# CPJKU/beat_this

Hardware: NVIDIA H100
Metric: clips/sec (30 s audio->beats, final0) (higher is better)
Workload: dtype f16

## Files before the change

beat_this_b200/csrc/kernels_attn.cu:

```cuda
#include <cstdio>
#include <type_traits>

#include "tc_common.cuh"

namespace bt {

constexpr int AT_BQ = 128;
constexpr int AT_BKV = 64;
constexpr int AT_NST = 4;
constexpr int AT_WARPS = 4;
constexpr int AT_RB = 2;
constexpr int AT_THREADS = 32 * AT_WARPS;
constexpr int AT_SQ = AT_BQ * 64;
constexpr int AT_SKV = AT_BKV * 64;
constexpr int AT_SMEM = 1024 + AT_SQ + AT_NST * 2 * AT_SKV + 128;
static_assert(AT_BQ == AT_WARPS * AT_RB * 16, "every query row of the tile belongs to one row block");

constexpr uint32_t AT_POLY_MASK = 0x52u;

__device__ __forceinline__ uint32_t sw64_off(int r, int c) {
  return static_cast<uint32_t>(r * 64 + ((c ^ ((r >> 1) & 3)) << 4));
}

__global__ void __launch_bounds__(AT_THREADS, 3)
attn_time_kernel(const __grid_constant__ CUtensorMap tmQ, const __grid_constant__ CUtensorMap tmKV,
                 const float* __restrict__ gates, h16* __restrict__ out, int L, int heads,
                 const ChunkSrc* __restrict__ chunks, int seqs_per_chunk) {
  extern __shared__ uint8_t smem_raw[];
  const uint32_t sbase = (smem_u32(smem_raw) + 1023u) & ~1023u;
  const uint32_t sQ = sbase;
  const uint32_t sK = sQ + AT_SQ;
  const uint32_t sV = sK + AT_NST * AT_SKV;
  const uint32_t bar_q = sV + AT_NST * AT_SKV;
  const uint32_t full = bar_q + 8;
  const uint32_t empty = full + 8 * AT_NST;

  const int warp = threadIdx.x >> 5, lane = threadIdx.x & 31;
  const int q0 = blockIdx.x * AT_BQ;
  const int h = blockIdx.y;
  const int seq = blockIdx.z;
  const int C = heads * 32;
  const int Lk = chunks ? chunks[seq / seqs_per_chunk].len : L;
  const int nkv = ceil_div(Lk, AT_BKV);

  if (threadIdx.x == 0) {
    mbar_init(bar_q, 1);
    for (int i = 0; i < AT_NST; ++i) {
      mbar_init(full + 8 * i, 1);
      mbar_init(empty + 8 * i, AT_WARPS);
    }
    fence_barrier_init();
  }
  __syncthreads();

  auto load_tile = [&](int t) {
    const int st = t % AT_NST;
    mbar_expect_tx(full + 8 * st, 2 * AT_SKV);
    tma_load_3d(sK + st * AT_SKV, &tmKV, full + 8 * st, C + h * 32, t * AT_BKV, seq);
    tma_load_3d(sV + st * AT_SKV, &tmKV, full + 8 * st, 2 * C + h * 32, t * AT_BKV, seq);
  };
  if (threadIdx.x == 0) {
    tma_prefetch_desc(&tmQ);
    tma_prefetch_desc(&tmKV);
    mbar_expect_tx(bar_q, AT_SQ);
    tma_load_3d(sQ, &tmQ, bar_q, h * 32, q0, seq);
    for (int t = 0; t < nkv && t < AT_NST; ++t) load_tile(t);
  }

  const int r0 = warp * (AT_RB * 16);
  mbar_wait(bar_q, 0);

  uint32_t qa[AT_RB][2][4];
#pragma unroll
  for (int b = 0; b < AT_RB; ++b)
#pragma unroll
    for (int ks = 0; ks < 2; ++ks)
      ldmatrix_x4(sQ + sw64_off(r0 + 16 * b + (lane & 15), 2 * ks + (lane >> 4)), qa[b][ks]);

  const uint32_t k_addr0 = sK + sw64_off(lane & 7, lane >> 3);
  const uint32_t v_addr0[2] = {sV + sw64_off(lane & 15, lane >> 4), sV + sw64_off(lane & 15, 2 + (lane >> 4))};
  const int key_lane = 2 * (lane & 3);

  float o[AT_RB][4][4];
#pragma unroll
  for (int b = 0; b < AT_RB; ++b)
#pragma unroll
    for (int d = 0; d < 4; ++d) o[b][d][0] = o[b][d][1] = o[b][d][2] = o[b][d][3] = 0.f;
  float m_run[AT_RB][2], l_run[AT_RB][2];
#pragma unroll
  for (int b = 0; b < AT_RB; ++b) m_run[b][0] = m_run[b][1] = -INFINITY, l_run[b][0] = l_run[b][1] = 0.f;
  auto kv_step = [&](uint32_t stage, uint32_t phase, auto last, int lim) {
    mbar_wait(full + stage / (AT_SKV / 8), phase);
    const uint32_t ka = k_addr0 + stage, va0 = v_addr0[0] + stage, va1 = v_addr0[1] + stage;
    float s[AT_RB][8][4];
#pragma unroll
    for (int nb = 0; nb < 8; ++nb) {
      uint32_t kf[4];
      ldmatrix_x4(ka + nb * 512, kf);
#pragma unroll
      for (int b = 0; b < AT_RB; ++b) {
        s[b][nb][0] = s[b][nb][1] = s[b][nb][2] = s[b][nb][3] = 0.f;
        mma_16816(s[b][nb], qa[b][0], kf[0], kf[1]);
        mma_16816(s[b][nb], qa[b][1], kf[2], kf[3]);
      }
    }
    if constexpr (decltype(last)::value) {
#pragma unroll
      for (int nb = 0; nb < 8; ++nb) {
        const int key = nb * 8 + key_lane;
#pragma unroll
        for (int b = 0; b < AT_RB; ++b) {
          if (key >= lim) s[b][nb][0] = s[b][nb][2] = -INFINITY;
          if (key + 1 >= lim) s[b][nb][1] = s[b][nb][3] = -INFINITY;
        }
      }
    }
    float mref[AT_RB][2];
#pragma unroll
    for (int b = 0; b < AT_RB; ++b) {
      float mx[2];
#pragma unroll
      for (int r = 0; r < 2; ++r) {
        float t[8];
#pragma unroll
        for (int nb = 0; nb < 8; ++nb) t[nb] = fmaxf(s[b][nb][2 * r], s[b][nb][2 * r + 1]);
#pragma unroll
        for (int w = 4; w > 0; w >>= 1)
#pragma unroll
          for (int i = 0; i < w; ++i) t[i] = fmaxf(t[i], t[i + w]);
        mx[r] = t[0];
      }
      float alpha[2];
#pragma unroll
      for (int r = 0; r < 2; ++r) {
        mx[r] = fmaxf(mx[r], __shfl_xor_sync(0xffffffffu, mx[r], 1));
        mx[r] = fmaxf(mx[r], __shfl_xor_sync(0xffffffffu, mx[r], 2));
        mref[b][r] = fmaxf(m_run[b][r], mx[r]);
        alpha[r] = ex2_approx(m_run[b][r] - mref[b][r]);
        m_run[b][r] = mref[b][r];
        l_run[b][r] *= alpha[r];
      }
#pragma unroll
      for (int d = 0; d < 4; ++d) {
        o[b][d][0] *= alpha[0]; o[b][d][1] *= alpha[0];
        o[b][d][2] *= alpha[1]; o[b][d][3] *= alpha[1];
      }
    }
    uint32_t pa[AT_RB][4][4];
#pragma unroll
    for (int b = 0; b < AT_RB; ++b)
#pragma unroll
      for (int nb = 0; nb < 8; ++nb) {
        float p[4];
#pragma unroll
        for (int i = 0; i < 4; ++i) {
          const float x = s[b][nb][i] - mref[b][i >> 1];
          p[i] = ((AT_POLY_MASK >> nb) & 1u) ? ex2_poly(x) : ex2_approx(x);
        }
        l_run[b][0] += p[0] + p[1];
        l_run[b][1] += p[2] + p[3];
        pa[b][nb >> 1][(nb & 1) * 2] = pack_h16x2(p[0], p[1]);
        pa[b][nb >> 1][(nb & 1) * 2 + 1] = pack_h16x2(p[2], p[3]);
      }
#pragma unroll
    for (int kk = 0; kk < 4; ++kk) {
#pragma unroll
      for (int dp = 0; dp < 2; ++dp) {
        uint32_t vf[4];
        ldmatrix_x4_trans((dp ? va1 : va0) + kk * 1024, vf);
#pragma unroll
        for (int b = 0; b < AT_RB; ++b) {
          mma_16816(o[b][2 * dp], pa[b][kk], vf[0], vf[1]);
          mma_16816(o[b][2 * dp + 1], pa[b][kk], vf[2], vf[3]);
        }
      }
    }
    __syncwarp();
    if (lane == 0) mbar_arrive(empty + stage / (AT_SKV / 8));
  };
  uint32_t stage = 0, phase = 0;
  for (int j = 0; j < nkv - 1; ++j) {
    if (threadIdx.x == 0 && j > 0 && j + AT_NST - 1 < nkv) {
      mbar_wait(empty + 8 * ((j - 1) % AT_NST), ((j - 1) / AT_NST) & 1);
      load_tile(j + AT_NST - 1);
    }
    kv_step(stage, phase, std::false_type{}, 0);
    stage += AT_SKV;
    if (stage == AT_NST * AT_SKV) stage = 0, phase ^= 1;
  }
  if (nkv > 0) kv_step(stage, phase, std::true_type{}, Lk - (nkv - 1) * AT_BKV);
#pragma unroll
  for (int b = 0; b < AT_RB; ++b)
#pragma unroll
    for (int r = 0; r < 2; ++r) {
      l_run[b][r] += __shfl_xor_sync(0xffffffffu, l_run[b][r], 1);
      l_run[b][r] += __shfl_xor_sync(0xffffffffu, l_run[b][r], 2);
    }
#pragma unroll
  for (int b = 0; b < AT_RB; ++b)
#pragma unroll
    for (int r = 0; r < 2; ++r) {
      const int q = q0 + r0 + 16 * b + (lane >> 2) + 8 * r;
      if (q < L) {
        const int64_t m = static_cast<int64_t>(seq) * L + q;
        const float gsc = gates[m * heads + h] / l_run[b][r];
        h16* dst = out + m * C + h * 32 + 2 * (lane & 3);
#pragma unroll
        for (int d = 0; d < 4; ++d)
          *reinterpret_cast<uint32_t*>(dst + 8 * d) = pack_h16x2(o[b][d][2 * r] * gsc, o[b][d][2 * r + 1] * gsc);
      }
    }
}

struct TcAttnPlan {
  CUtensorMap tmQ;
  CUtensorMap tmKV;
  int seqs, L, heads;
};

TcAttnPlan* tc_attn_plan_create(const void* qkv, int seqs, int L, int heads, char* err, int errlen) {
  TcAttnPlan* p = new TcAttnPlan();
  p->seqs = seqs; p->L = L; p->heads = heads;
  const int C = heads * 32;
  const uint64_t dims[3] = {static_cast<uint64_t>(3 * C), static_cast<uint64_t>(L), static_cast<uint64_t>(seqs)};
  const uint64_t strides[2] = {static_cast<uint64_t>(3 * C) * 2, static_cast<uint64_t>(L) * 3 * C * 2};
  const uint32_t box_q[3] = {32, AT_BQ, 1};
  const uint32_t box_kv[3] = {32, AT_BKV, 1};
  if (!make_tmap(&p->tmQ, qkv, 3, dims, strides, box_q, 64, err, errlen) ||
      !make_tmap(&p->tmKV, qkv, 3, dims, strides, box_kv, 64, err, errlen)) {
    delete p;
    return nullptr;
  }
  return p;
}
void tc_attn_plan_destroy(TcAttnPlan* p) { delete p; }

void launch_attn_time_tc(const TcAttnPlan* p, const float* gates, void* out, cudaStream_t st, const ChunkSrc* chunks,
                         int seqs_per_chunk) {
  dim3 grid(ceil_div(p->L, AT_BQ), p->heads, p->seqs);
  attn_time_kernel<<<grid, AT_THREADS, AT_SMEM, st>>>(p->tmQ, p->tmKV, gates, reinterpret_cast<h16*>(out), p->L, p->heads,
                                                      chunks, seqs_per_chunk);
}

int tc_init_attn(char* err, int errlen) {
  const cudaError_t r = cudaFuncSetAttribute(attn_time_kernel, cudaFuncAttributeMaxDynamicSharedMemorySize, AT_SMEM);
  if (r != cudaSuccess) {
    snprintf(err, errlen, "cudaFuncSetAttribute(attn_time_kernel) failed: %s", cudaGetErrorString(r));
    return -1;
  }
  return 0;
}

}
```

beat_this_b200/csrc/tc_common.cuh:

```cuda
#pragma once
#include <cuda.h>

#include "epilogue.cuh"

namespace bt {

__device__ __forceinline__ void tma_store_3d(const void* tmap, uint32_t smem_src, int32_t c0, int32_t c1, int32_t c2) {
  asm volatile("cp.async.bulk.tensor.3d.global.shared::cta.bulk_group [%0, {%2, %3, %4}], [%1];" ::"l"(
                   reinterpret_cast<uint64_t>(tmap)),
               "r"(smem_src), "r"(c0), "r"(c1), "r"(c2)
               : "memory");
}
__device__ __forceinline__ void bulk_commit() { asm volatile("cp.async.bulk.commit_group;" ::: "memory"); }
template <int N>
__device__ __forceinline__ void bulk_wait_read() {
  asm volatile("cp.async.bulk.wait_group.read %0;" ::"n"(N) : "memory");
}
__device__ __forceinline__ void named_bar_sync(int id, int count) {
  asm volatile("bar.sync %0, %1;" ::"r"(id), "r"(count) : "memory");
}
__device__ __forceinline__ void stmatrix_x4(uint32_t addr, uint32_t r0, uint32_t r1, uint32_t r2, uint32_t r3) {
  asm volatile("stmatrix.sync.aligned.m8n8.x4.shared.b16 [%0], {%1, %2, %3, %4};" ::"r"(addr), "r"(r0), "r"(r1), "r"(r2),
               "r"(r3)
               : "memory");
}
__device__ __forceinline__ float2 ld_shared_v2_f32(uint32_t addr) {
  float2 q;
  asm volatile("ld.shared.v2.f32 {%0, %1}, [%2];" : "=f"(q.x), "=f"(q.y) : "r"(addr) : "memory");
  return q;
}
__device__ __forceinline__ void st_shared_v2_f32(uint32_t addr, float x, float y) {
  asm volatile("st.shared.v2.f32 [%0], {%1, %2};" ::"r"(addr), "f"(x), "f"(y) : "memory");
}

__device__ __forceinline__ float ex2_approx(float x) {
  float y;
  asm("ex2.approx.ftz.f32 %0, %1;" : "=f"(y) : "f"(x));
  return y;
}
__device__ __forceinline__ float ex2_poly(float x) {
  x = fmaxf(x, -120.0f);
  const float magic = 12582912.0f;
  const float t = x + magic;
  const float r = x - (t - magic);
  float p = fmaf(0.05508868f, r, 0.24260405f);
  p = fmaf(p, r, 0.69327623f);
  p = fmaf(p, r, 0.99992895f);
  int y;
  asm("mad.lo.s32 %0, %1, 8388608, %2;" : "=r"(y) : "r"(__float_as_int(t)), "r"(__float_as_int(p)));
  return __int_as_float(y);
}

template <int SW>
__device__ __forceinline__ uint64_t make_wgmma_desc(uint32_t smem_addr) {
  static_assert(SW == 128 || SW == 64, "swizzle");
  constexpr uint64_t layout = SW == 128 ? 1 : 2;
  constexpr uint64_t sbo = (8 * SW) >> 4;
  return static_cast<uint64_t>((smem_addr & 0x3FFFF) >> 4) | (1ull << 16) | (sbo << 32) | (layout << 62);
}
__device__ __forceinline__ void wgmma_fence() { asm volatile("wgmma.fence.sync.aligned;" ::: "memory"); }
__device__ __forceinline__ void wgmma_commit() { asm volatile("wgmma.commit_group.sync.aligned;" ::: "memory"); }
template <int N>
__device__ __forceinline__ void wgmma_wait() {
  asm volatile("wgmma.wait_group.sync.aligned %0;" ::"n"(N) : "memory");
}
template <int R>
__device__ __forceinline__ void setmaxnreg_dec() {
  asm volatile("setmaxnreg.dec.sync.aligned.u32 %0;" ::"n"(R));
}
template <int R>
__device__ __forceinline__ void setmaxnreg_inc() {
  asm volatile("setmaxnreg.inc.sync.aligned.u32 %0;" ::"n"(R));
}
template <int N>
__device__ __forceinline__ void wgmma_m64k16(float (&d)[N / 2], uint64_t a_desc, uint64_t b_desc, uint32_t accumulate) {
  static_assert(N == 32 || N == 64 || N == 128 || N == 192 || N == 256, "wgmma width");
  if constexpr (N == 32) {
    asm volatile(
        "{\n\t.reg .pred p;\n\tsetp.ne.b32 p, %18, 0;\n\t"
        "wgmma.mma_async.sync.aligned.m64n32k16.f32." BT_H16_MMA_SYNC " "
        "{%0, %1, %2, %3, %4, %5, %6, %7, %8, %9, %10, %11, %12, %13, %14, %15}, "
        "%16, %17, p, 1, 1, 0, 0;\n\t}"
        : "+f"(d[0]), "+f"(d[1]), "+f"(d[2]), "+f"(d[3]), "+f"(d[4]), "+f"(d[5]), "+f"(d[6]), "+f"(d[7]),
          "+f"(d[8]), "+f"(d[9]), "+f"(d[10]), "+f"(d[11]), "+f"(d[12]), "+f"(d[13]), "+f"(d[14]), "+f"(d[15])
        : "l"(a_desc), "l"(b_desc), "r"(accumulate)
        : "memory");
  } else if constexpr (N == 64) {
    asm volatile(
        "{\n\t.reg .pred p;\n\tsetp.ne.b32 p, %34, 0;\n\t"
        "wgmma.mma_async.sync.aligned.m64n64k16.f32." BT_H16_MMA_SYNC " "
        "{%0, %1, %2, %3, %4, %5, %6, %7, %8, %9, %10, %11, %12, %13, %14, %15, %16, %17, %18, %19, %20, %21, %22, %23, %24, %25, %26, %27, %28, %29, %30, %31}, "
        "%32, %33, p, 1, 1, 0, 0;\n\t}"
        : "+f"(d[0]), "+f"(d[1]), "+f"(d[2]), "+f"(d[3]), "+f"(d[4]), "+f"(d[5]), "+f"(d[6]), "+f"(d[7]),
          "+f"(d[8]), "+f"(d[9]), "+f"(d[10]), "+f"(d[11]), "+f"(d[12]), "+f"(d[13]), "+f"(d[14]), "+f"(d[15]),
          "+f"(d[16]), "+f"(d[17]), "+f"(d[18]), "+f"(d[19]), "+f"(d[20]), "+f"(d[21]), "+f"(d[22]), "+f"(d[23]),
          "+f"(d[24]), "+f"(d[25]), "+f"(d[26]), "+f"(d[27]), "+f"(d[28]), "+f"(d[29]), "+f"(d[30]), "+f"(d[31])
        : "l"(a_desc), "l"(b_desc), "r"(accumulate)
        : "memory");
  } else if constexpr (N == 128) {
    asm volatile(
        "{\n\t.reg .pred p;\n\tsetp.ne.b32 p, %66, 0;\n\t"
        "wgmma.mma_async.sync.aligned.m64n128k16.f32." BT_H16_MMA_SYNC " "
        "{%0, %1, %2, %3, %4, %5, %6, %7, %8, %9, %10, %11, %12, %13, %14, %15, %16, %17, %18, %19, %20, %21, %22, %23, %24, %25, %26, %27, %28, %29, %30, %31, %32, %33, %34, %35, %36, %37, %38, %39, %40, %41, %42, %43, %44, %45, %46, %47, %48, %49, %50, %51, %52, %53, %54, %55, %56, %57, %58, %59, %60, %61, %62, %63}, "
        "%64, %65, p, 1, 1, 0, 0;\n\t}"
        : "+f"(d[0]), "+f"(d[1]), "+f"(d[2]), "+f"(d[3]), "+f"(d[4]), "+f"(d[5]), "+f"(d[6]), "+f"(d[7]),
          "+f"(d[8]), "+f"(d[9]), "+f"(d[10]), "+f"(d[11]), "+f"(d[12]), "+f"(d[13]), "+f"(d[14]), "+f"(d[15]),
          "+f"(d[16]), "+f"(d[17]), "+f"(d[18]), "+f"(d[19]), "+f"(d[20]), "+f"(d[21]), "+f"(d[22]), "+f"(d[23]),
          "+f"(d[24]), "+f"(d[25]), "+f"(d[26]), "+f"(d[27]), "+f"(d[28]), "+f"(d[29]), "+f"(d[30]), "+f"(d[31]),
          "+f"(d[32]), "+f"(d[33]), "+f"(d[34]), "+f"(d[35]), "+f"(d[36]), "+f"(d[37]), "+f"(d[38]), "+f"(d[39]),
          "+f"(d[40]), "+f"(d[41]), "+f"(d[42]), "+f"(d[43]), "+f"(d[44]), "+f"(d[45]), "+f"(d[46]), "+f"(d[47]),
          "+f"(d[48]), "+f"(d[49]), "+f"(d[50]), "+f"(d[51]), "+f"(d[52]), "+f"(d[53]), "+f"(d[54]), "+f"(d[55]),
          "+f"(d[56]), "+f"(d[57]), "+f"(d[58]), "+f"(d[59]), "+f"(d[60]), "+f"(d[61]), "+f"(d[62]), "+f"(d[63])
        : "l"(a_desc), "l"(b_desc), "r"(accumulate)
        : "memory");
  } else if constexpr (N == 192) {
    asm volatile(
        "{\n\t.reg .pred p;\n\tsetp.ne.b32 p, %98, 0;\n\t"
        "wgmma.mma_async.sync.aligned.m64n192k16.f32." BT_H16_MMA_SYNC " "
        "{%0, %1, %2, %3, %4, %5, %6, %7, %8, %9, %10, %11, %12, %13, %14, %15, %16, %17, %18, %19, %20, %21, %22, %23, %24, %25, %26, %27, %28, %29, %30, %31, %32, %33, %34, %35, %36, %37, %38, %39, %40, %41, %42, %43, %44, %45, %46, %47, %48, %49, %50, %51, %52, %53, %54, %55, %56, %57, %58, %59, %60, %61, %62, %63, %64, %65, %66, %67, %68, %69, %70, %71, %72, %73, %74, %75, %76, %77, %78, %79, %80, %81, %82, %83, %84, %85, %86, %87, %88, %89, %90, %91, %92, %93, %94, %95}, "
        "%96, %97, p, 1, 1, 0, 0;\n\t}"
        : "+f"(d[0]), "+f"(d[1]), "+f"(d[2]), "+f"(d[3]), "+f"(d[4]), "+f"(d[5]), "+f"(d[6]), "+f"(d[7]),
          "+f"(d[8]), "+f"(d[9]), "+f"(d[10]), "+f"(d[11]), "+f"(d[12]), "+f"(d[13]), "+f"(d[14]), "+f"(d[15]),
          "+f"(d[16]), "+f"(d[17]), "+f"(d[18]), "+f"(d[19]), "+f"(d[20]), "+f"(d[21]), "+f"(d[22]), "+f"(d[23]),
          "+f"(d[24]), "+f"(d[25]), "+f"(d[26]), "+f"(d[27]), "+f"(d[28]), "+f"(d[29]), "+f"(d[30]), "+f"(d[31]),
          "+f"(d[32]), "+f"(d[33]), "+f"(d[34]), "+f"(d[35]), "+f"(d[36]), "+f"(d[37]), "+f"(d[38]), "+f"(d[39]),
          "+f"(d[40]), "+f"(d[41]), "+f"(d[42]), "+f"(d[43]), "+f"(d[44]), "+f"(d[45]), "+f"(d[46]), "+f"(d[47]),
          "+f"(d[48]), "+f"(d[49]), "+f"(d[50]), "+f"(d[51]), "+f"(d[52]), "+f"(d[53]), "+f"(d[54]), "+f"(d[55]),
          "+f"(d[56]), "+f"(d[57]), "+f"(d[58]), "+f"(d[59]), "+f"(d[60]), "+f"(d[61]), "+f"(d[62]), "+f"(d[63]),
          "+f"(d[64]), "+f"(d[65]), "+f"(d[66]), "+f"(d[67]), "+f"(d[68]), "+f"(d[69]), "+f"(d[70]), "+f"(d[71]),
          "+f"(d[72]), "+f"(d[73]), "+f"(d[74]), "+f"(d[75]), "+f"(d[76]), "+f"(d[77]), "+f"(d[78]), "+f"(d[79]),
          "+f"(d[80]), "+f"(d[81]), "+f"(d[82]), "+f"(d[83]), "+f"(d[84]), "+f"(d[85]), "+f"(d[86]), "+f"(d[87]),
          "+f"(d[88]), "+f"(d[89]), "+f"(d[90]), "+f"(d[91]), "+f"(d[92]), "+f"(d[93]), "+f"(d[94]), "+f"(d[95])
        : "l"(a_desc), "l"(b_desc), "r"(accumulate)
        : "memory");
  } else if constexpr (N == 256) {
    asm volatile(
        "{\n\t.reg .pred p;\n\tsetp.ne.b32 p, %130, 0;\n\t"
        "wgmma.mma_async.sync.aligned.m64n256k16.f32." BT_H16_MMA_SYNC " "
        "{%0, %1, %2, %3, %4, %5, %6, %7, %8, %9, %10, %11, %12, %13, %14, %15, %16, %17, %18, %19, %20, %21, %22, %23, %24, %25, %26, %27, %28, %29, %30, %31, %32, %33, %34, %35, %36, %37, %38, %39, %40, %41, %42, %43, %44, %45, %46, %47, %48, %49, %50, %51, %52, %53, %54, %55, %56, %57, %58, %59, %60, %61, %62, %63, %64, %65, %66, %67, %68, %69, %70, %71, %72, %73, %74, %75, %76, %77, %78, %79, %80, %81, %82, %83, %84, %85, %86, %87, %88, %89, %90, %91, %92, %93, %94, %95, %96, %97, %98, %99, %100, %101, %102, %103, %104, %105, %106, %107, %108, %109, %110, %111, %112, %113, %114, %115, %116, %117, %118, %119, %120, %121, %122, %123, %124, %125, %126, %127}, "
        "%128, %129, p, 1, 1, 0, 0;\n\t}"
        : "+f"(d[0]), "+f"(d[1]), "+f"(d[2]), "+f"(d[3]), "+f"(d[4]), "+f"(d[5]), "+f"(d[6]), "+f"(d[7]),
          "+f"(d[8]), "+f"(d[9]), "+f"(d[10]), "+f"(d[11]), "+f"(d[12]), "+f"(d[13]), "+f"(d[14]), "+f"(d[15]),
          "+f"(d[16]), "+f"(d[17]), "+f"(d[18]), "+f"(d[19]), "+f"(d[20]), "+f"(d[21]), "+f"(d[22]), "+f"(d[23]),
          "+f"(d[24]), "+f"(d[25]), "+f"(d[26]), "+f"(d[27]), "+f"(d[28]), "+f"(d[29]), "+f"(d[30]), "+f"(d[31]),
          "+f"(d[32]), "+f"(d[33]), "+f"(d[34]), "+f"(d[35]), "+f"(d[36]), "+f"(d[37]), "+f"(d[38]), "+f"(d[39]),
          "+f"(d[40]), "+f"(d[41]), "+f"(d[42]), "+f"(d[43]), "+f"(d[44]), "+f"(d[45]), "+f"(d[46]), "+f"(d[47]),
          "+f"(d[48]), "+f"(d[49]), "+f"(d[50]), "+f"(d[51]), "+f"(d[52]), "+f"(d[53]), "+f"(d[54]), "+f"(d[55]),
          "+f"(d[56]), "+f"(d[57]), "+f"(d[58]), "+f"(d[59]), "+f"(d[60]), "+f"(d[61]), "+f"(d[62]), "+f"(d[63]),
          "+f"(d[64]), "+f"(d[65]), "+f"(d[66]), "+f"(d[67]), "+f"(d[68]), "+f"(d[69]), "+f"(d[70]), "+f"(d[71]),
          "+f"(d[72]), "+f"(d[73]), "+f"(d[74]), "+f"(d[75]), "+f"(d[76]), "+f"(d[77]), "+f"(d[78]), "+f"(d[79]),
          "+f"(d[80]), "+f"(d[81]), "+f"(d[82]), "+f"(d[83]), "+f"(d[84]), "+f"(d[85]), "+f"(d[86]), "+f"(d[87]),
          "+f"(d[88]), "+f"(d[89]), "+f"(d[90]), "+f"(d[91]), "+f"(d[92]), "+f"(d[93]), "+f"(d[94]), "+f"(d[95]),
          "+f"(d[96]), "+f"(d[97]), "+f"(d[98]), "+f"(d[99]), "+f"(d[100]), "+f"(d[101]), "+f"(d[102]), "+f"(d[103]),
          "+f"(d[104]), "+f"(d[105]), "+f"(d[106]), "+f"(d[107]), "+f"(d[108]), "+f"(d[109]), "+f"(d[110]), "+f"(d[111]),
          "+f"(d[112]), "+f"(d[113]), "+f"(d[114]), "+f"(d[115]), "+f"(d[116]), "+f"(d[117]), "+f"(d[118]), "+f"(d[119]),
          "+f"(d[120]), "+f"(d[121]), "+f"(d[122]), "+f"(d[123]), "+f"(d[124]), "+f"(d[125]), "+f"(d[126]), "+f"(d[127])
        : "l"(a_desc), "l"(b_desc), "r"(accumulate)
        : "memory");
  }
}

__device__ __forceinline__ void mma_16816(float (&d)[4], const uint32_t (&a)[4], uint32_t b0, uint32_t b1) {
  asm volatile("mma.sync.aligned.m16n8k16.row.col.f32." BT_H16_MMA_SYNC ".f32 {%0, %1, %2, %3}, {%4, %5, %6, %7}, {%8, %9}, "
               "{%0, %1, %2, %3};"
               : "+f"(d[0]), "+f"(d[1]), "+f"(d[2]), "+f"(d[3])
               : "r"(a[0]), "r"(a[1]), "r"(a[2]), "r"(a[3]), "r"(b0), "r"(b1));
}
__device__ __forceinline__ void ldmatrix_x4(uint32_t addr, uint32_t (&r)[4]) {
  asm volatile("ldmatrix.sync.aligned.m8n8.x4.shared.b16 {%0, %1, %2, %3}, [%4];"
               : "=r"(r[0]), "=r"(r[1]), "=r"(r[2]), "=r"(r[3])
               : "r"(addr)
               : "memory");
}
__device__ __forceinline__ void ldmatrix_x4_trans(uint32_t addr, uint32_t (&r)[4]) {
  asm volatile("ldmatrix.sync.aligned.m8n8.x4.trans.shared.b16 {%0, %1, %2, %3}, [%4];"
               : "=r"(r[0]), "=r"(r[1]), "=r"(r[2]), "=r"(r[3])
               : "r"(addr)
               : "memory");
}

extern int g_num_sms;
bool make_tmap(CUtensorMap* tm, const void* base, int rank, const uint64_t* dims, const uint64_t* strides_bytes,
               const uint32_t* box, int swizzle_bytes, char* err, int errlen);
int tc_init_attn(char* err, int errlen);
int tc_init_attn_freq(char* err, int errlen);
int tc_init_fused(char* err, int errlen);

}
```

Baseline: 815.7.

## Port time-attention kernel from mma.sync to pipelined wgmma warpgroups

Rewrites the flash-attention time kernel to use two warpgroups issuing asynchronous wgmma, computing QK^T from shared-memory descriptors and PV with register-sourced P. Score MMAs for the next KV tile are issued before the softmax of the current one, so tensor-core work overlaps the exponentials. The empty-barrier release moves to one arrival per warpgroup, and the final division uses a custom f64-refined reciprocal. This adds register pressure from double-buffered scores and depends on the wgmma descriptor and swizzle layout matching the TMA layout.

```diff
diff --git a/beat_this_b200/csrc/kernels_attn.cu b/beat_this_b200/csrc/kernels_attn.cu
--- a/beat_this_b200/csrc/kernels_attn.cu
+++ b/beat_this_b200/csrc/kernels_attn.cu
@@ -8,21 +8,35 @@
 constexpr int AT_BQ = 128;
 constexpr int AT_BKV = 64;
 constexpr int AT_NST = 4;
-constexpr int AT_WARPS = 4;
-constexpr int AT_RB = 2;
-constexpr int AT_THREADS = 32 * AT_WARPS;
+constexpr int AT_WG = 2;
+constexpr int AT_THREADS = 128 * AT_WG;
 constexpr int AT_SQ = AT_BQ * 64;
 constexpr int AT_SKV = AT_BKV * 64;
 constexpr int AT_SMEM = 1024 + AT_SQ + AT_NST * 2 * AT_SKV + 128;
-static_assert(AT_BQ == AT_WARPS * AT_RB * 16, "every query row of the tile belongs to one row block");
+static_assert(AT_BQ == AT_WG * 64, "every query row of the tile belongs to one warpgroup");
 
 constexpr uint32_t AT_POLY_MASK = 0x52u;
 
-__device__ __forceinline__ uint32_t sw64_off(int r, int c) {
-  return static_cast<uint32_t>(r * 64 + ((c ^ ((r >> 1) & 3)) << 4));
-}
-
-__global__ void __launch_bounds__(AT_THREADS, 3)
+__device__ __forceinline__ float div_rn_nocall(float a, float b) {
+  const double ad = a, bd = b;
+  double y;
+  asm("rcp.approx.ftz.f64 %0, %1;" : "=d"(y) : "d"(bd));
+  y = fma(y, fma(-bd, y, 1.0), y);
+  y = fma(y, fma(-bd, y, 1.0), y);
+  const double q = ad * y;
+  return static_cast<float>(fma(fma(-bd, q, ad), y, q));
+}
+
+__device__ __forceinline__ void mbar_wait_asm(uint32_t bar, uint32_t parity) {
+  asm volatile(
+      "{\n\t.reg .pred p;\n\tWAIT_%=:\n\t"
+      "mbarrier.try_wait.parity.shared::cta.b64 p, [%0], %1;\n\t"
+      "@!p bra WAIT_%=;\n\t}" ::"r"(bar),
+      "r"(parity)
+      : "memory");
+}
+
+__global__ void __launch_bounds__(AT_THREADS, 2)
 attn_time_kernel(const __grid_constant__ CUtensorMap tmQ, const __grid_constant__ CUtensorMap tmKV,
                  const float* __restrict__ gates, h16* __restrict__ out, int L, int heads,
                  const ChunkSrc* __restrict__ chunks, int seqs_per_chunk) {
@@ -35,7 +49,8 @@
   const uint32_t full = bar_q + 8;
   const uint32_t empty = full + 8 * AT_NST;
 
-  const int warp = threadIdx.x >> 5, lane = threadIdx.x & 31;
+  const int wg = threadIdx.x >> 7, warp = (threadIdx.x >> 5) & 3, lane = threadIdx.x & 31;
+  const bool leader = (threadIdx.x & 127) == 0;
   const int q0 = blockIdx.x * AT_BQ;
   const int h = blockIdx.y;
   const int seq = blockIdx.z;
@@ -47,7 +62,7 @@
     mbar_init(bar_q, 1);
     for (int i = 0; i < AT_NST; ++i) {
       mbar_init(full + 8 * i, 1);
-      mbar_init(empty + 8 * i, AT_WARPS);
+      mbar_init(empty + 8 * i, AT_WG);
     }
     fence_barrier_init();
   }
@@ -67,149 +82,141 @@
     for (int t = 0; t < nkv && t < AT_NST; ++t) load_tile(t);
   }
 
-  const int r0 = warp * (AT_RB * 16);
+  const uint32_t sQw = sQ + wg * 64 * 64;
+  const int key_lane = 2 * (lane & 3);
   mbar_wait(bar_q, 0);
 
-  uint32_t qa[AT_RB][2][4];
-#pragma unroll
-  for (int b = 0; b < AT_RB; ++b)
-#pragma unroll
-    for (int ks = 0; ks < 2; ++ks)
-      ldmatrix_x4(sQ + sw64_off(r0 + 16 * b + (lane & 15), 2 * ks + (lane >> 4)), qa[b][ks]);
-
-  const uint32_t k_addr0 = sK + sw64_off(lane & 7, lane >> 3);
-  const uint32_t v_addr0[2] = {sV + sw64_off(lane & 15, lane >> 4), sV + sw64_off(lane & 15, 2 + (lane >> 4))};
-  const int key_lane = 2 * (lane & 3);
-
-  float o[AT_RB][4][4];
-#pragma unroll
-  for (int b = 0; b < AT_RB; ++b)
-#pragma unroll
-    for (int d = 0; d < 4; ++d) o[b][d][0] = o[b][d][1] = o[b][d][2] = o[b][d][3] = 0.f;
-  float m_run[AT_RB][2], l_run[AT_RB][2];
-#pragma unroll
-  for (int b = 0; b < AT_RB; ++b) m_run[b][0] = m_run[b][1] = -INFINITY, l_run[b][0] = l_run[b][1] = 0.f;
-  auto kv_step = [&](uint32_t stage, uint32_t phase, auto last, int lim) {
-    mbar_wait(full + stage / (AT_SKV / 8), phase);
-    const uint32_t ka = k_addr0 + stage, va0 = v_addr0[0] + stage, va1 = v_addr0[1] + stage;
-    float s[AT_RB][8][4];
-#pragma unroll
-    for (int nb = 0; nb < 8; ++nb) {
-      uint32_t kf[4];
-      ldmatrix_x4(ka + nb * 512, kf);
-#pragma unroll
-      for (int b = 0; b < AT_RB; ++b) {
-        s[b][nb][0] = s[b][nb][1] = s[b][nb][2] = s[b][nb][3] = 0.f;
-        mma_16816(s[b][nb], qa[b][0], kf[0], kf[1]);
-        mma_16816(s[b][nb], qa[b][1], kf[2], kf[3]);
-      }
-    }
-    if constexpr (decltype(last)::value) {
+  float s[2][32], o[16];
+#pragma unroll
+  for (int i = 0; i < 16; ++i) asm volatile("mov.b32 %0, 0;" : "=f"(o[i]));
+  uint32_t pa[2][4][4];
+  float m_run[2] = {-INFINITY, -INFINITY}, l_run[2] = {0.f, 0.f};
+
+  const uint64_t qdesc = make_wgmma_desc<64>(sQw), kdesc = make_wgmma_desc<64>(sK);
+  auto issue_scores = [&](float (&acc)[32], uint32_t stage) {
+    wgmma_fence();
+    wgmma_m64n64k16_zero(acc, qdesc, kdesc + (stage >> 4));
+    wgmma_m64k16<64>(acc, qdesc + 2, kdesc + (stage >> 4) + 2, 1u);
+  };
+  auto kv_step = [&](int j, uint32_t stage, uint32_t phase, auto B, auto last, int lim) {
+    constexpr int b = decltype(B)::value;
+    constexpr bool is_last = decltype(last)::value;
+    if constexpr (!is_last) {
+      const uint32_t next = stage + AT_SKV == AT_NST * AT_SKV ? 0u : stage + AT_SKV;
+      mbar_wait(full + next / (AT_SKV / 8), next == 0 ? phase ^ 1u : phase);
+      issue_scores(s[b ^ 1], next);
+      wgmma_commit();
+    }
+    wgmma_wait<is_last ? 1 : 2>();
+    wgmma_fence_operands(s[b]);
+    if constexpr (is_last) {
 #pragma unroll
       for (int nb = 0; nb < 8; ++nb) {
         const int key = nb * 8 + key_lane;
-#pragma unroll
-        for (int b = 0; b < AT_RB; ++b) {
-          if (key >= lim) s[b][nb][0] = s[b][nb][2] = -INFINITY;
-          if (key + 1 >= lim) s[b][nb][1] = s[b][nb][3] = -INFINITY;
-        }
-      }
-    }
-    float mref[AT_RB][2];
-#pragma unroll
-    for (int b = 0; b < AT_RB; ++b) {
-      float mx[2];
-#pragma unroll
-      for (int r = 0; r < 2; ++r) {
-        float t[8];
-#pragma unroll
-        for (int nb = 0; nb < 8; ++nb) t[nb] = fmaxf(s[b][nb][2 * r], s[b][nb][2 * r + 1]);
-#pragma unroll
-        for (int w = 4; w > 0; w >>= 1)
-#pragma unroll
-          for (int i = 0; i < w; ++i) t[i] = fmaxf(t[i], t[i + w]);
-        mx[r] = t[0];
-      }
-      float alpha[2];
-#pragma unroll
-      for (int r = 0; r < 2; ++r) {
-        mx[r] = fmaxf(mx[r], __shfl_xor_sync(0xffffffffu, mx[r], 1));
-        mx[r] = fmaxf(mx[r], __shfl_xor_sync(0xffffffffu, mx[r], 2));
-        mref[b][r] = fmaxf(m_run[b][r], mx[r]);
-        alpha[r] = ex2_approx(m_run[b][r] - mref[b][r]);
-        m_run[b][r] = mref[b][r];
-        l_run[b][r] *= alpha[r];
-      }
-#pragma unroll
-      for (int d = 0; d < 4; ++d) {
-        o[b][d][0] *= alpha[0]; o[b][d][1] *= alpha[0];
-        o[b][d][2] *= alpha[1]; o[b][d][3] *= alpha[1];
-      }
-    }
-    uint32_t pa[AT_RB][4][4];
-#pragma unroll
-    for (int b = 0; b < AT_RB; ++b)
-#pragma unroll
-      for (int nb = 0; nb < 8; ++nb) {
-        float p[4];
-#pragma unroll
-        for (int i = 0; i < 4; ++i) {
-          const float x = s[b][nb][i] - mref[b][i >> 1];
-          p[i] = ((AT_POLY_MASK >> nb) & 1u) ? ex2_poly(x) : ex2_approx(x);
-        }
-        l_run[b][0] += p[0] + p[1];
-        l_run[b][1] += p[2] + p[3];
-        pa[b][nb >> 1][(nb & 1) * 2] = pack_h16x2(p[0], p[1]);
-        pa[b][nb >> 1][(nb & 1) * 2 + 1] = pack_h16x2(p[2], p[3]);
-      }
-#pragma unroll
-    for (int kk = 0; kk < 4; ++kk) {
-#pragma unroll
-      for (int dp = 0; dp < 2; ++dp) {
-        uint32_t vf[4];
-        ldmatrix_x4_trans((dp ? va1 : va0) + kk * 1024, vf);
-#pragma unroll
-        for (int b = 0; b < AT_RB; ++b) {
-          mma_16816(o[b][2 * dp], pa[b][kk], vf[0], vf[1]);
-          mma_16816(o[b][2 * dp + 1], pa[b][kk], vf[2], vf[3]);
-        }
-      }
+        if (key >= lim) s[b][4 * nb] = s[b][4 * nb + 2] = -INFINITY;
+        if (key + 1 >= lim) s[b][4 * nb + 1] = s[b][4 * nb + 3] = -INFINITY;
+      }
+    }
+    float mref[2], alpha[2];
+#pragma unroll
+    for (int r = 0; r < 2; ++r) {
+      float t[8];
+#pragma unroll
+      for (int nb = 0; nb < 8; ++nb) t[nb] = fmaxf(s[b][4 * nb + 2 * r], s[b][4 * nb + 2 * r + 1]);
+#pragma unroll
+      for (int w = 4; w > 0; w >>= 1)
+#pragma unroll
+        for (int i = 0; i < w; ++i) t[i] = fmaxf(t[i], t[i + w]);
+      float mx = t[0];
+      mx = fmaxf(mx, __shfl_xor_sync(0xffffffffu, mx, 1));
+      mx = fmaxf(mx, __shfl_xor_sync(0xffffffffu, mx, 2));
+      mref[r] = fmaxf(m_run[r], mx);
+      alpha[r] = ex2_approx(m_run[r] - mref[r]);
+      m_run[r] = mref[r];
+      l_run[r] *= alpha[r];
+    }
+    wgmma_wait<is_last ? 0 : 1>();
+    wgmma_fence_operands(o);
+    if (leader && j > 0) mbar_arrive(empty + 8 * ((j - 1) % AT_NST));
+#pragma unroll
+    for (int d = 0; d < 4; ++d) {
+      o[4 * d] *= alpha[0]; o[4 * d + 1] *= alpha[0];
+      o[4 * d + 2] *= alpha[1]; o[4 * d + 3] *= alpha[1];
+    }
+#pragma unroll
+    for (int nb = 0; nb < 8; ++nb) {
+      float p[4];
+#pragma unroll
+      for (int i = 0; i < 4; ++i) {
+        const float x = s[b][4 * nb + i] - mref[i >> 1];
+        p[i] = ((AT_POLY_MASK >> nb) & 1u) ? ex2_poly(x) : ex2_approx(x);
+      }
+      l_run[0] += p[0] + p[1];
+      l_run[1] += p[2] + p[3];
+      pa[b][nb >> 1][(nb & 1) * 2] = pack_h16x2(p[0], p[1]);
+      pa[b][nb >> 1][(nb & 1) * 2 + 1] = pack_h16x2(p[2], p[3]);
+    }
+    wgmma_fence_operands(o);
+#pragma unroll
+    for (int kk = 0; kk < 4; ++kk) wgmma_fence_operands(pa[b][kk]);
+    wgmma_fence();
+#pragma unroll
+    for (int kk = 0; kk < 4; ++kk)
+      wgmma_m64n32k16_rs_tb(o, pa[b][kk], kdesc + ((AT_NST * AT_SKV + stage + kk * 1024) >> 4));
+    wgmma_commit();
+    if constexpr (is_last) {
+      wgmma_wait<0>();
+      wgmma_fence_operands(o);
+    }
+    if (threadIdx.x == 0 && j > 0 && j + AT_NST - 1 < nkv) {
+      mbar_wait_asm(empty + 8 * ((j - 1) % AT_NST), ((j - 1) / AT_NST) & 1);
+      load_tile(j + AT_NST - 1);
     }
     __syncwarp();
-    if (lane == 0) mbar_arrive(empty + stage / (AT_SKV / 8));
   };
-  uint32_t stage = 0, phase = 0;
-  for (int j = 0; j < nkv - 1; ++j) {
-    if (threadIdx.x == 0 && j > 0 && j + AT_NST - 1 < nkv) {
-      mbar_wait(empty + 8 * ((j - 1) % AT_NST), ((j - 1) / AT_NST) & 1);
-      load_tile(j + AT_NST - 1);
-    }
-    kv_step(stage, phase, std::false_type{}, 0);
-    stage += AT_SKV;
-    if (stage == AT_NST * AT_SKV) stage = 0, phase ^= 1;
-  }
-  if (nkv > 0) kv_step(stage, phase, std::true_type{}, Lk - (nkv - 1) * AT_BKV);
-#pragma unroll
-  for (int b = 0; b < AT_RB; ++b)
-#pragma unroll
-    for (int r = 0; r < 2; ++r) {
-      l_run[b][r] += __shfl_xor_sync(0xffffffffu, l_run[b][r], 1);
-      l_run[b][r] += __shfl_xor_sync(0xffffffffu, l_run[b][r], 2);
-    }
-#pragma unroll
-  for (int b = 0; b < AT_RB; ++b)
-#pragma unroll
-    for (int r = 0; r < 2; ++r) {
-      const int q = q0 + r0 + 16 * b + (lane >> 2) + 8 * r;
-      if (q < L) {
-        const int64_t m = static_cast<int64_t>(seq) * L + q;
-        const float gsc = gates[m * heads + h] / l_run[b][r];
-        h16* dst = out + m * C + h * 32 + 2 * (lane & 3);
-#pragma unroll
-        for (int d = 0; d < 4; ++d)
-          *reinterpret_cast<uint32_t*>(dst + 8 * d) = pack_h16x2(o[b][d][2 * r] * gsc, o[b][d][2 * r + 1] * gsc);
-      }
-    }
+  if (nkv > 0) {
+    mbar_wait(full, 0);
+    issue_scores(s[0], 0);
+    wgmma_commit();
+    wgmma_commit();
+    using B0 = std::integral_constant<int, 0>;
+    using B1 = std::integral_constant<int, 1>;
+    const int lim = Lk - (nkv - 1) * AT_BKV;
+    uint32_t stage = 0, phase = 0;
+    for (int j = 0;; j += 2) {
+      if (j + 1 == nkv) {
+        kv_step(j, stage, phase, B0{}, std::true_type{}, lim);
+        break;
+      }
+      kv_step(j, stage, phase, B0{}, std::false_type{}, 0);
+      stage += AT_SKV;
+      if (stage == AT_NST * AT_SKV) stage = 0, phase ^= 1;
+      if (j + 2 == nkv) {
+        kv_step(j + 1, stage, phase, B1{}, std::true_type{}, lim);
+        break;
+      }
+      kv_step(j + 1, stage, phase, B1{}, std::false_type{}, 0);
+      stage += AT_SKV;
+      if (stage == AT_NST * AT_SKV) stage = 0, phase ^= 1;
+    }
+  }
+#pragma unroll
+  for (int r = 0; r < 2; ++r) {
+    l_run[r] += __shfl_xor_sync(0xffffffffu, l_run[r], 1);
+    l_run[r] += __shfl_xor_sync(0xffffffffu, l_run[r], 2);
+  }
+#pragma unroll
+  for (int r = 0; r < 2; ++r) {
+    const int q = q0 + 64 * wg + 16 * warp + (lane >> 2) + 8 * r;
+    if (q < L) {
+      const int64_t m = static_cast<int64_t>(seq) * L + q;
+      const float gsc = div_rn_nocall(gates[m * heads + h], l_run[r]);
+      h16* dst = out + m * C + h * 32 + 2 * (lane & 3);
+#pragma unroll
+      for (int d = 0; d < 4; ++d)
+        *reinterpret_cast<uint32_t*>(dst + 8 * d) = pack_h16x2(o[4 * d + 2 * r] * gsc, o[4 * d + 2 * r + 1] * gsc);
+    }
+  }
 }
 
 struct TcAttnPlan {
diff --git a/beat_this_b200/csrc/tc_common.cuh b/beat_this_b200/csrc/tc_common.cuh
--- a/beat_this_b200/csrc/tc_common.cuh
+++ b/beat_this_b200/csrc/tc_common.cuh
@@ -160,6 +160,39 @@
   }
 }
 
+__device__ __forceinline__ void wgmma_m64n64k16_zero(float (&d)[32], uint64_t a_desc, uint64_t b_desc) {
+  asm volatile(
+      "wgmma.mma_async.sync.aligned.m64n64k16.f32." BT_H16_MMA_SYNC " "
+      "{%0, %1, %2, %3, %4, %5, %6, %7, %8, %9, %10, %11, %12, %13, %14, %15, %16, %17, %18, %19, %20, %21, %22, %23, %24, %25, %26, %27, %28, %29, %30, %31}, "
+      "%32, %33, 0, 1, 1, 0, 0;"
+      : "=f"(d[0]), "=f"(d[1]), "=f"(d[2]), "=f"(d[3]), "=f"(d[4]), "=f"(d[5]), "=f"(d[6]), "=f"(d[7]),
+        "=f"(d[8]), "=f"(d[9]), "=f"(d[10]), "=f"(d[11]), "=f"(d[12]), "=f"(d[13]), "=f"(d[14]), "=f"(d[15]),
+        "=f"(d[16]), "=f"(d[17]), "=f"(d[18]), "=f"(d[19]), "=f"(d[20]), "=f"(d[21]), "=f"(d[22]), "=f"(d[23]),
+        "=f"(d[24]), "=f"(d[25]), "=f"(d[26]), "=f"(d[27]), "=f"(d[28]), "=f"(d[29]), "=f"(d[30]), "=f"(d[31])
+      : "l"(a_desc), "l"(b_desc)
+      : "memory");
+}
+__device__ __forceinline__ void wgmma_m64n32k16_rs_tb(float (&d)[16], const uint32_t (&a)[4], uint64_t b_desc) {
+  asm volatile(
+      "wgmma.mma_async.sync.aligned.m64n32k16.f32." BT_H16_MMA_SYNC " "
+      "{%0, %1, %2, %3, %4, %5, %6, %7, %8, %9, %10, %11, %12, %13, %14, %15}, "
+      "{%16, %17, %18, %19}, %20, 1, 1, 1, 1;"
+      : "+f"(d[0]), "+f"(d[1]), "+f"(d[2]), "+f"(d[3]), "+f"(d[4]), "+f"(d[5]), "+f"(d[6]), "+f"(d[7]),
+        "+f"(d[8]), "+f"(d[9]), "+f"(d[10]), "+f"(d[11]), "+f"(d[12]), "+f"(d[13]), "+f"(d[14]), "+f"(d[15])
+      : "r"(a[0]), "r"(a[1]), "r"(a[2]), "r"(a[3]), "l"(b_desc)
+      : "memory");
+}
+template <int N>
+__device__ __forceinline__ void wgmma_fence_operands(float (&r)[N]) {
+#pragma unroll
+  for (int i = 0; i < N; ++i) asm volatile("" : "+f"(r[i])::"memory");
+}
+template <int N>
+__device__ __forceinline__ void wgmma_fence_operands(uint32_t (&r)[N]) {
+#pragma unroll
+  for (int i = 0; i < N; ++i) asm volatile("" : "+r"(r[i])::"memory");
+}
+
 __device__ __forceinline__ void mma_16816(float (&d)[4], const uint32_t (&a)[4], uint32_t b0, uint32_t b1) {
   asm volatile("mma.sync.aligned.m16n8k16.row.col.f32." BT_H16_MMA_SYNC ".f32 {%0, %1, %2, %3}, {%4, %5, %6, %7}, {%8, %9}, "
                "{%0, %1, %2, %3};"
```

New measurement: 836.3 (median of 6 runs). +2.5%, better.
